# sakarias88/racer-tracer

Measured on AMD Instinct MI355X. Metric: Msamples/s (W*H*spp/s) at 1920x1080, higher is better.
Workload: dtype f64; 1 GPU; cornell_box.yml 1920x1080 1024spp max_depth 20; strip_rows=8, parallelism=image rows interleaved over 1 GPU(s)

## Files before the change

racer-tracer_amd/csrc/rt_pool_lds.h:

```cpp
#pragma once
#include "rt_trace_common.h"

namespace RT_KNS {

struct NoiseSlots {
    double p[8][3];
    int depth[8];
    int perlin[8];
    double term[8][8];
};
struct alignas(16) Req4 {
    uint32_t x, y, z, w;
};
struct alignas(8) SphereSlot {
    uint32_t b, y, x, w, z, base;
};
static_assert(sizeof(SphereSlot) == 3 * sizeof(double), "a slot holds the request or the sample");

template <bool TEXTURED> union SamplerScratch {
    Req4 req[32];
    SphereSlot sphere[32];
    NoiseSlots noise;
};
template <> union SamplerScratch<false> {
    Req4 req[32];
    SphereSlot sphere[32];
};

struct alignas(16) ItemInfo {
    int chunk, tx, ty, tile_py0, region, reg_tiles, rows_aligned, _pad;
};

template <bool TEXTURED, int NBUF, bool OVERLAP> struct WaveLds {
    double base[OVERLAP ? 1 : 64][3];
    double u[OVERLAP ? 64 : 1];
    double sum[OVERLAP ? 128 : 64][3];
    SamplerScratch<TEXTURED> scratch;
    uint8_t pix_of[64];
    double v[NBUF][64];
    ItemInfo info[2];
    double ulc[3];
};

enum : uint32_t { RING_SLOTS = 92u };
struct PretraceLds {
    double cam_origin[3], bg_top[3];
    double u[64];
    double sum[64][3];
    SamplerScratch<false> scratch;
    uint8_t pix_of[64];
    double ring_v[RING_SLOTS];
    double ring_t[RING_SLOTS];
    uint32_t ring_w[RING_SLOTS];
    uint16_t ring_best[RING_SLOTS];
    uint32_t n_started;
    uint32_t rect_mask;
    ItemInfo info[1];
    double ulc[3];
};

}
```

racer-tracer_amd/csrc/rt_trace_common.h:

```cpp
#pragma once
#include <hip/hip_runtime.h>
#include <stdint.h>
#include "rt_device_types.h"
#include "rt_bvh_slab.h"
#include "../../include/rt_abi.h"
#include "../../include/rt_rng.h"

#ifdef RT_EXACT_DIV
#define RT_KNS rtdev_exact
#define RT_LAUNCHER(name) name##_exact
#else
#define RT_KNS rtdev_fast
#define RT_LAUNCHER(name) name
#endif

namespace RT_KNS {
using namespace rtdev;

#define RT_CONSTANT __attribute__((address_space(4)))
__device__ __forceinline__ Prim load_prim_uniform(const Prim *table, int i) {
    Prim p;
    __builtin_memcpy(&p, (const RT_CONSTANT Prim *)(table + i), sizeof(Prim));
    return p;
}
// ... 340 lines not shown
#ifndef RT_EXACT_DIV
        return box_slab_t(P.p, o, d, inv_d, t_min, t_max, t_out, aux);
#endif
        bool any = false;
        double closest = t_max;
#pragma unroll
        for (int s = 0; s < 6; ++s) {
            int axis;
            double a0, a1, b0, b1, k, t;
            box_side(P.p, s, axis, a0, a1, b0, b1, k);
            if (rect_t<false>(axis, a0, a1, b0, b1, k, o, d, inv_d, t_min, closest, t)) {
                closest = t;
                aux = s;
                any = true;
            }
        }
        t_out = closest;
        return any;
    }
    }
}

__device__ __forceinline__ bool box_t(const Prim &P, d3 o, d3 d, d3 inv_d, double t_min, double t_max, double &t_out, int &side) {
#ifdef RT_EXACT_DIV
    return prim_t<PRIMS_ANY>(P, o, d, inv_d, 0.0, 0.0, t_min, t_max, t_out, side);
#else
#ifndef RT_BOX_LOADS_LAZY
    asm volatile("; box record requested" ::"s"(P.p[0]), "s"(P.p[1]), "s"(P.p[2]), "s"(P.p[3]), "s"(P.p[4]), "s"(P.p[5]), "s"(P.rot_sin),
                 "s"(P.rot_cos), "s"(P.tr[0]), "s"(P.tr[1]), "s"(P.tr[2]), "s"(P.flags));
#endif
    o = o - ld3(P.tr);
    if (P.flags & RT_PRIM_HAS_ROTATE_Y) {
        o = rot_fwd(o, P.rot_sin, P.rot_cos);
        d = rot_fwd(d, P.rot_sin, P.rot_cos);
        inv_d.x = rcp_f64(d.x);
        inv_d.z = rcp_f64(d.z);
    }
    return box_slab_t(P.p, o, d, inv_d, t_min, t_max, t_out, side);
#endif
}

__device__ __forceinline__ const BvhNode *bvh_nodes_for(const TraceArgs &A, d3 d) {
    if (A.bvh_nodes_ordered == nullptr) return A.bvh_nodes;
    const int oct = (d.x < 0.0 ? 1 : 0) | (d.y < 0.0 ? 2 : 0) | (d.z < 0.0 ? 4 : 0);
    return A.bvh_nodes_ordered + (size_t)oct * (size_t)(A.n_bvh_nodes + 1);
}

struct NoMark {
    __device__ __forceinline__ void operator()(int) const {}
};
template <int PRIMS, class Mark = NoMark>
__device__ __forceinline__ void closest_hit_bvh(const TraceArgs &A, const BvhNode *nodes, d3 o, d3 d, d3 inv_d,
                                                double inv_a, double time, double t_min, double &best_t, int &best,
                                                int &best_aux, unsigned *walk_stats = nullptr, Mark mark = Mark()) {
    const RT_CONSTANT TraceArgs *K = kernargs_here();
    double t0 = 0.0;
    {
        const double ax = (K->bvh_root_mn[0] - o.x) * inv_d.x, bx = (K->bvh_root_mx[0] - o.x) * inv_d.x;
        const double ay = (K->bvh_root_mn[1] - o.y) * inv_d.y, by = (K->bvh_root_mx[1] - o.y) * inv_d.y;
        const double az = (K->bvh_root_mn[2] - o.z) * inv_d.z, bz = (K->bvh_root_mx[2] - o.z) * inv_d.z;
        const double t_enter = fmax(fmax(fmin(ax, bx), fmin(ay, by)), fmin(az, bz));
        const double t_exit = fmin(fmin(fmax(ax, bx), fmax(ay, by)), fmin(fmax(az, bz), best_t));
        if (!(fmax(t_enter, t_min) <= t_exit)) return;
        if (t_enter > 0.0) t0 = t_enter;
    }
    const SlabRay sr = slab_ray((float)(fma(t0, d.x, o.x) - K->bvh_center[0]), (float)(fma(t0, d.y, o.y) - K->bvh_center[1]),
                                (float)(fma(t0, d.z, o.z) - K->bvh_center[2]), inv_d.x, inv_d.y, inv_d.z);
    const float slack = 0x1p-20f;
    const float tmin_f = (float)(t_min - t0) - fabsf((float)(t_min - t0)) * slack - 0x1p-126f;
    auto far_of = [&](double bt) {
        const float f = (float)(bt - t0);
        return fmaxf(f + fabsf(f) * slack, tmin_f);
    };
    float best_f = far_of(best_t);
    if (!(tmin_f <= best_f)) return;
    typedef float f2 __attribute__((ext_vector_type(2)));
    const f2 p01 = {sr.ivx, sr.ivy}, p23 = {sr.ivz, sr.nox}, p45 = {sr.noy, sr.noz};
    int i = 0;
    const int n = A.n_bvh_nodes;
    while (i < n) {
        int fc = 0;
        for (;;) {
            if (walk_stats) ++walk_stats[0];
            const uint4 *raw = reinterpret_cast<const uint4 *>(&nodes[i]);
            const uint4 q0 = raw[0], q1 = raw[1];
            const f2 qx = {__uint_as_float(q0.x), __uint_as_float(q0.y)}, qy = {__uint_as_float(q0.z), __uint_as_float(q0.w)},
                     qz = {__uint_as_float(q1.x), __uint_as_float(q1.y)};
            f2 tx, ty, tz;
            float nx, ny, nz, fx, fy, fz, t_near, t_far;
            asm("v_pk_fma_f32 %0, %1, %2, %3 op_sel:[0,0,1] op_sel_hi:[1,0,1]" : "=v"(tx) : "v"(qx), "v"(p01), "v"(p23));
            asm("v_pk_fma_f32 %0, %1, %2, %3 op_sel:[0,1,0] op_sel_hi:[1,1,0]" : "=v"(ty) : "v"(qy), "v"(p01), "v"(p45));
            asm("v_pk_fma_f32 %0, %1, %2, %3 op_sel:[0,0,1] op_sel_hi:[1,0,1]" : "=v"(tz) : "v"(qz), "v"(p23), "v"(p45));
            asm("v_min_f32 %0, %8, %9\n\tv_max_f32 %1, %8, %9\n\t"
                "v_min_f32 %2, %10, %11\n\tv_max_f32 %3, %10, %11\n\t"
                "v_min_f32 %4, %12, %13\n\tv_max_f32 %5, %12, %13\n\t"
                "v_max_f32 %4, %4, %14\n\tv_min_f32 %5, %5, %15\n\t"
                "v_max3_f32 %6, %0, %2, %4\n\tv_min3_f32 %7, %1, %3, %5"
                : "=&v"(nx), "=&v"(fx), "=&v"(ny), "=&v"(fy), "=&v"(nz), "=&v"(fz), "=&v"(t_near), "=&v"(t_far)
                : "v"(tx.x), "v"(tx.y), "v"(ty.x), "v"(ty.y), "v"(tz.x), "v"(tz.y), "v"(tmin_f), "v"(best_f));
            const bool hit = !(t_near > t_far);
            fc = (int)q1.w;
            i = hit ? i + 1 : (int)q1.z;
            if (hit && fc != 0) break;
        }
        const int count = fc & 7, first = fc >> 3;
        mark(11);
        bool improved = false;
        for (int k = 0; k < count; ++k) {
            if (walk_stats) ++walk_stats[1];
            const int pi = first + k;
            double t;
            int aux = 0;
            bool hit;
            const LeafGeo &G = A.leaf_geo[pi];
            const long long tag = G.tag;
            const d3 center = ld3(G.c0) + ((time - A.leaf_time_a) * A.leaf_inv_dt) * ld3(G.dc);
            hit = sphere_t(center, G.radius2, o, d, inv_a, t_min, best_t, t) && tag == 0;
            if (tag != 0) hit = prim_t<PRIMS>(A.prims[pi], o, d, inv_d, inv_a, time, t_min, best_t, t, aux);
            if (hit) {
                best_t = t;
                best = pi;
                best_aux = aux;
                improved = true;
            }
        }
        if (improved) best_f = far_of(best_t);
        mark(12);
    }
}

struct UV {
    double u, v;
};
__device__ __noinline__ UV sphere_uv(d3 outward) {
    const double PI = 3.14159265358979323846;
    double theta = acos(-outward.y);
    double phi = atan2(-outward.z, outward.x) + PI;
#ifdef RT_EXACT_DIV
    return UV{phi / (2.0 * PI), theta / PI};
#else
    return UV{phi * (1.0 / (2.0 * PI)), theta * (1.0 / PI)};
#endif
}

#define RT_UV_EPS_U 5e-7
#define RT_UV_EPS_V 2e-6
__device__ __forceinline__ UV sphere_uv_f32(d3 outward) {
    const float theta = acosf(-(float)outward.y);
    const float phi = atan2f(-(float)outward.z, (float)outward.x);
    return UV{((double)phi + 3.14159265358979323846) * (1.0 / (2.0 * 3.14159265358979323846)),
              (double)theta * (1.0 / 3.14159265358979323846)};
}

template <int PRIMS, bool TEXTURED, bool FAST_UV = false>
__device__ __forceinline__ Hit prim_hit_record(const Prim &P, d3 o, d3 d, double time, double t, int aux, bool want_uv) {
    d3 oo = o, dd = d;
    const int flags = PRIMS == PRIMS_ANY ? P.flags : 0;
    if (flags & RT_PRIM_HAS_TRANSLATE) oo = oo - ld3(P.tr);
    if (flags & RT_PRIM_HAS_ROTATE_Y) {
        oo = rot_fwd(oo, P.rot_sin, P.rot_cos);
        dd = rot_fwd(dd, P.rot_sin, P.rot_cos);
    }
    Hit h;
    h.point = oo + t * dd;
    h.u = 0.0;
    h.v = 0.0;
    h.uv_approx = false;
    const int kind = PRIMS == PRIMS_SPHERES ? (int)RT_PRIM_SPHERE : P.kind;
    if (PRIMS == PRIMS_ANY && kind == RT_PRIM_MOVING_SPHERE) {
        const d3 center = ld3(P.p) + ((time - P.rot_sin) * P.rot_cos) * ld3(P.tr);
        d3 outward = (h.point - center) * P.inv_radius;
        if (TEXTURED && want_uv) {
            const UV uv = sphere_uv(h.point);
            h.u = uv.u;
            h.v = uv.v;
        }
        set_face_normal(h, dd, outward);
    } else if (PRIMS != PRIMS_RECTS && kind == RT_PRIM_SPHERE) {
        d3 outward = (h.point - ld3(P.p)) * P.inv_radius;
        if (TEXTURED && want_uv) {
#ifndef RT_EXACT_DIV
            if (FAST_UV && flags == 0 && fma(-outward.y, outward.y, 1.0) >= 0x1p-10) {
                const UV uv = sphere_uv_f32(outward);
                h.u = uv.u;
                h.v = uv.v;
                h.uv_approx = true;
            } else
#endif
            {
                const UV uv = sphere_uv(outward);
                h.u = uv.u;
                h.v = uv.v;
            }
        }
        set_face_normal(h, dd, outward);
    } else {
        int axis;
        double a0, a1, b0, b1, k;
        if (PRIMS == PRIMS_ANY && kind == RT_PRIM_BOX) {
            box_side(P.p, aux, axis, a0, a1, b0, b1, k);
        } else {
            axis = kind == RT_PRIM_XY_RECT ? 2 : (kind == RT_PRIM_XZ_RECT ? 1 : 0);
            a0 = P.p[0]; a1 = P.p[1]; b0 = P.p[2]; b1 = P.p[3];
        }
        if (TEXTURED && want_uv) {
            int ia = axis == 0 ? 1 : 0;
            int ib = axis == 2 ? 1 : 2;
            h.u = (comp(h.point, ia) - a0) / (a1 - a0);
            h.v = (comp(h.point, ib) - b0) / (b1 - b0);
        }
        set_face_normal_axis(h, dd, axis);
    }
    if (flags & RT_PRIM_HAS_ROTATE_Y) {
        h.point = rot_back(h.point, P.rot_sin, P.rot_cos);
        set_face_normal(h, dd, rot_back(h.normal, P.rot_sin, P.rot_cos));
    }
    if (flags & RT_PRIM_HAS_TRANSLATE) {
        h.point = h.point + ld3(P.tr);
        set_face_normal(h, d, h.normal);
    }
    return h;
}

template <bool IDENTITY>
__device__ __forceinline__ double perlin_noise(const Perlin &pl, d3 p) {
    double fx = floor(p.x), fy = floor(p.y), fz = floor(p.z);
    double u = p.x - fx, v = p.y - fy, w = p.z - fz;
    int i = (int)fx, j = (int)fy, k = (int)fz;
    double uu = u * u * (3.0 - 2.0 * u);
    double vv = v * v * (3.0 - 2.0 * v);
    double ww = w * w * (3.0 - 2.0 * w);
    const double fu[2] = {1.0 - uu, uu}, fv[2] = {1.0 - vv, vv}, fw[2] = {1.0 - ww, ww};
    double accum = 0.0;
#pragma unroll
    for (int di = 0; di < 2; ++di)
#pragma unroll
        for (int dj = 0; dj < 2; ++dj) {
            const double fuv = fu[di] * fv[dj];
#pragma unroll
            for (int dk = 0; dk < 2; ++dk) {
                int index;
                if (IDENTITY)
                    index = (i + di) ^ (j + dj) ^ (k + dk);
                else
                    index = pl.perm_x[(uint32_t)(i + di) & 255u] ^ pl.perm_y[(uint32_t)(j + dj) & 255u] ^
                            pl.perm_z[(uint32_t)(k + dk) & 255u];
                const double *g = pl.ranvec[index & 255];
                d3 weight = mk(u - di, v - dj, w - dk);
                accum += fuv * fw[dk] * dot(ld3(g), weight);
            }
        }
    return accum;
}

template <bool IDENTITY>
__device__ __forceinline__ double perlin_turbulence(const Perlin &pl, d3 p, int depth) {
    double accum = 0.0, weight = 1.0;
    for (int o = 0; o < depth; ++o) {
        accum += weight * perlin_noise<IDENTITY>(pl, p);
        weight *= 0.5;
        p = p * 2.0;
    }
    return fabs(accum);
}

__device__ __forceinline__ double clamp01(double x) { return x < 0.0 ? 0.0 : (x > 1.0 ? 1.0 : x); }

__device__ __forceinline__ double sin_lean(double x) {
    const double kd = rint(x * 0.63661977236758134308);
    double r = fma(-kd, 1.57079632673412561417e+00, x);
    r = fma(-kd, 6.07710050630396597660e-11, r);
    r = fma(-kd, 2.02226624871116645580e-21, r);
    const int q = (int)kd;
    const double z = r * r;
    const double ps = fma(z, fma(z, fma(z, fma(z, 1.58969099521155010221e-10, -2.50507602534068634195e-08),
                                        2.75573137070700676789e-06), -1.98412698298579493134e-04),
                          8.33333333332248946124e-03);
    const double sn = fma(z * r, fma(z, ps, -1.66666666666666324348e-01), r);
    const double pc = fma(z, fma(z, fma(z, fma(z, fma(z, -1.13596475577881948265e-11, 2.08757232129817482790e-09),
                                               -2.75573143513906633035e-07), 2.48015872894767294178e-05),
                                 -1.38888888888741095749e-03), 4.16666666666666019037e-02);
    const double cs = 1.0 - fma(0.5, z, -(z * z) * pc);
    const double v = (q & 1) ? cs : sn;
    return (q & 2) ? -v : v;
}

__device__ __forceinline__ int sin_sign(double x) {
    const double kd = rint(x * 0.63661977236758134308);
    double r = fma(-kd, 1.57079632673412561417e+00, x);
    r = fma(-kd, 6.07710050630396597660e-11, r);
    r = fma(-kd, 2.02226624871116645580e-21, r);
    const int q = (int)kd;
    const int s = (q & 1) ? 1 : (r > 0.0 ? 1 : (r < 0.0 ? -1 : 0));
    return (q & 2) ? -s : s;
}

__device__ __forceinline__ bool sines_product_negative(double a, double b, double c) {
#ifndef RT_EXACT_DIV
    const double inv_pi = 0.31830988618379067154;
    const uint32_t odd = (uint32_t)(int)floor(a * inv_pi) ^ (uint32_t)(int)floor(b * inv_pi) ^ (uint32_t)(int)floor(c * inv_pi);
    const bool zero = a * b * c == 0.0;
    return !zero && (odd & 1u) != 0u;
#else
    uint32_t negative = 0;
    bool zero = false;
    const double xs[3] = {a, b, c};
#pragma unroll
    for (int k = 0; k < 3; ++k) {
        const double kd = rint(xs[k] * 0.63661977236758134308);
        double r = fma(-kd, 1.57079632673412561417e+00, xs[k]);
        r = fma(-kd, 6.07710050630396597660e-11, r);
        r = fma(-kd, 2.02226624871116645580e-21, r);
        const uint32_t q = (uint32_t)(int)kd;
        const uint32_t r_neg = (uint32_t)((unsigned long long)__double_as_longlong(r) >> 63);
        zero = zero || ((q & 1u) == 0u && r == 0.0);
        negative ^= (q >> 1) ^ (~q & r_neg);
    }
// ... 95 lines not shown
```

racer-tracer_amd/csrc/rt_trace_pool_kernel.hip:

```cpp
#include <cstddef>
#include <type_traits>
#include "rt_trace_common.h"
#include "rt_primary_bounds.h"
#include "rt_variant_dispatch.h"
#include "rt_pool_profile.h"
#include "rt_pool_lds.h"
#include "rt_pool_coop.h"
#include "rt_pool_deliver.h"

#ifndef RT_OCC_TEX
#define RT_OCC_TEX 4
#endif
#ifndef RT_OCC_TEX_BVH
#define RT_OCC_TEX_BVH 4
#endif
#ifndef RT_OCC_TEX_ANY
#define RT_OCC_TEX_ANY 4
#endif
#ifndef RT_OCC_SPEC
#define RT_OCC_SPEC 5
#endif
#ifndef RT_OCC_ANY
#define RT_OCC_ANY 5
#endif
// ... 171 lines not shown
        const uint64_t valid_mask = ballot(my_valid);
        n_valid = __popcll(valid_mask);
        bool culled = false;
        if constexpr (PRETRACE) {
            const RT_CONSTANT TraceArgs *K = kernargs_here();
            const int x0 = K->cull_px0, x1 = K->cull_px1, y0 = K->cull_py0, y1 = K->cull_py1;
            const uint64_t seen = valid_mask & ballot(my_px >= x0) & ballot(my_px <= x1) & ballot(my_py >= y0) & ballot(my_py <= y1);
            culled = seen == 0ull && K->bg.kind != RT_BG_SKY && K->max_depth >= 1;
            uint32_t rect_mask = ~0u;
            if (!culled) {
                const RT_CONSTANT rtdev::PrimaryRects *R = primary_rects_here();
                const int n_rects = R->n;
                for (int i = 0; i < n_rects; ++i) {
                    const int rx0 = R->r[i].px0, rx1 = R->r[i].px1, ry0 = R->r[i].py0, ry1 = R->r[i].py1;
                    const uint64_t sees = valid_mask & ballot(my_px >= rx0) & ballot(my_px <= rx1) & ballot(my_py >= ry0) & ballot(my_py <= ry1);
                    if (sees == 0ull) rect_mask &= ~(1u << i);
                }
            }
            if (lane == 0) L.rect_mask = rect_mask;
        }
        {
            if (!culled) {
                uint32_t pixel_stream = RT_RNG_SAMPLE_PIXEL;
                if constexpr (PRETRACE) asm volatile("" : "+s"(pixel_stream));
                PathRng prng{my_pixel, pixel_stream, A.seed_lo, A.seed_hi};
                u4 bj = prng.block(0, RT_RNG_PIXEL, 0);
                const RT_CONSTANT TraceArgs *K = kernargs_here();
                const double u = div_by((double)my_px + u53(bj.a, bj.b), (double)(A.width - 1), K->inv_width_m1);
                if constexpr (OVERLAP || PRETRACE) {
                    L.u[lane] = u;
                } else {
                    const d3 base = ld3(K->cam.ulc) + u * ld3(K->cam.horizontal);
                    L.base[lane][0] = base.x;
                    L.base[lane][1] = base.y;
                    L.base[lane][2] = base.z;
                }
            }
            unsigned long long zero = FIXED_SUMS ? 0ull - (unsigned long long)n_smp * 0x4330000000000000ull : 0ull;
            if constexpr (PRETRACE) asm volatile("" : "+v"(zero));
            unsigned long long *sum = reinterpret_cast<unsigned long long *>(L.sum[cur * 64 + lane]);
            sum[0] = zero;
            sum[1] = zero;
            sum[2] = zero;
            if (my_valid) L.pix_of[lane_rank(valid_mask)] = lane;
            if (lane == 0) L.info[cur] = ItemInfo{(int)chunk, tx, ty, tile_py0, region, (int)reg_tiles, rows_aligned ? 1 : 0, 0};
        }
        if constexpr (PRETRACE) {
            if (culled) {
                const d3 bg = ld3(L.bg_top);
                if (bg.x != 0.0 || bg.y != 0.0 || bg.z != 0.0)
                    for (int k = 0; k < n_smp; ++k) {
                        atomicAdd(&L.sum[lane_of_wave][0], bg.x);
                        atomicAdd(&L.sum[lane_of_wave][1], bg.y);
                        atomicAdd(&L.sum[lane_of_wave][2], bg.z);
                    }
                if (__builtin_amdgcn_inverse_ballot_w64(valid_mask)) n_segments += (unsigned int)n_smp;
                if (lane == 0) L.n_started += (uint32_t)n_valid * (uint32_t)n_smp;
            }
        }
        if (!rows_aligned) tile_py0 = -1;
        total = culled ? 0u : (uint32_t)n_valid * (uint32_t)n_smp;
        next = 0;
        n_batches = (total + 63u) >> 6;
        batches_done = 0;
        batch_due = n_batches > 0u ? 0u : ~0u;
        ring_head = 0;
        return true;
    };
    auto finish_item = [&](int s) {
        int lane = lane_of_wave;
        asm volatile("" : "+v"(lane));
        const ItemInfo I = L.info[s];
        const int chunk = __builtin_amdgcn_readfirstlane(I.chunk), f_tx = __builtin_amdgcn_readfirstlane(I.tx),
                  f_ty = __builtin_amdgcn_readfirstlane(I.ty), f_py0 = __builtin_amdgcn_readfirstlane(I.tile_py0);
        const bool f_aligned = __builtin_amdgcn_readfirstlane(I.rows_aligned) != 0;
        const int f_px = (f_tx * 8 + (lane & 7)) * A.step_x;
        const int f_vrow = f_ty * 8 + (lane >> 3);
        int f_py = f_py0 + (lane >> 3) * A.step_y;
        if (!f_aligned) f_py = ((f_vrow / A.strip_rows) * A.strip_count + A.strip_index) * A.strip_rows + f_vrow % A.strip_rows;
        const bool f_valid = f_px < A.cover_w && f_vrow < A.owned_rows && f_py < A.height;
        double s0 = L.sum[s * 64 + lane][0], s1 = L.sum[s * 64 + lane][1], s2 = L.sum[s * 64 + lane][2];
        if (FIXED_SUMS) {
            const double unscale = kernargs_here()->sum_unscale;
            s0 = (double)(unsigned long long)__double_as_longlong(s0) * unscale;
            s1 = (double)(unsigned long long)__double_as_longlong(s1) * unscale;
            s2 = (double)(unsigned long long)__double_as_longlong(s2) * unscale;
        }
        if (A.deliver_out == nullptr) {
            if (f_valid) {
                const size_t in_slice = (size_t)f_vrow * (size_t)A.width + (size_t)f_px;
                double *dst = A.partial + ((size_t)(A.chunk_base + chunk) * (size_t)A.slice_rows * (size_t)A.width + in_slice) * 3;
                dst[0] = s0;
                dst[1] = s1;
                dst[2] = s2;
            }
        } else {
            deliver_item(kernargs_here(), s0, s1, s2, f_valid, chunk, f_tx, f_ty, f_py0, f_aligned, __builtin_amdgcn_readfirstlane(I.region),
                         (uint32_t)__builtin_amdgcn_readfirstlane(I.reg_tiles));
        }
    };
    auto entry_of = [&](uint32_t w, int &py_out, uint32_t &pixel_out, uint32_t &sample_out, int &pix) {
        int s_off;
        if (n_valid == 64) {
            pix = (int)(w & 63u);
            s_off = (int)(w >> 6);
        } else {
            s_off = (int)(w / (uint32_t)n_valid);
            pix = L.pix_of[w - (uint32_t)s_off * (uint32_t)n_valid];
        }
        pixel_out = (uint32_t)shfl_i((int)my_pixel, pix);
        py_out = tile_py0 + (pix >> 3) * A.step_y;
        if (tile_py0 < 0) {
            const int vrow = __builtin_amdgcn_readfirstlane(L.info[(state >> 6) & 1u].ty) * 8 + (pix >> 3);
            py_out = ((vrow / A.strip_rows) * A.strip_count + A.strip_index) * A.strip_rows + vrow % A.strip_rows;
        }
        sample_out = (uint32_t)(smp0 + s_off);
    };
    auto prepare_batch = [&](uint32_t b) {
        if constexpr (!PRETRACE) {
        int lane = lane_of_wave;
        asm volatile("" : "+v"(lane));
        const RT_CONSTANT TraceArgs *K = kernargs_here();
        const uint32_t w = b * 64u + (uint32_t)lane;
        const bool in_pool = w < total;
        int py_b = 0;
        uint32_t pixel_b = 0, sample_b = 0;
        int pix_b = 0;
        entry_of(w, py_b, pixel_b, sample_b, pix_b);
        const u4 bc = philox4x32(pixel_b, sample_b, RT_RNG_CAMERA, 0u, A.seed_lo, A.seed_hi);
        const int buf = (int)(b & (uint32_t)(NBUF - 1));
        L.v[buf][lane] = div_by((double)py_b + u53(bc.a, bc.b), (double)(A.height - 1), K->inv_height_m1);
        if (PRIMS == PRIMS_ANY && ray_times != nullptr) ray_times[buf][lane] = K->cam.time_a + (K->cam.time_b - K->cam.time_a) * u53(bc.c, bc.d);
        if (K->cam.lens_radius != 0.0) {
            double lx = 0.0, ly = 0.0;
            coop_random_in_unit_disk(in_pool, pixel_b, sample_b, A.seed_lo, A.seed_hi, lane, L.scratch.req, lx, ly);
            lens[buf][lane][0] = lx * K->cam.lens_radius;
            lens[buf][lane][1] = ly * K->cam.lens_radius;
        }
        }
    };

    auto camera_ray = [&](int pix, double v, double lens_x, double lens_y, d3 &ro, d3 &rd) {
        if constexpr (PRETRACE) {
        const RT_CONSTANT TraceArgs *K = kernargs_here();
        ro = ld3(L.cam_origin);
        rd = (ld3(L.ulc) + L.u[pix] * ld3(K->cam.horizontal)) - v * ld3(K->cam.vertical) - ld3(K->cam.origin);
        if (kernargs_here()->lens_lds != 0) {
            const d3 offset = ld3(K->cam.right) * lens_x + ld3(K->cam.up) * lens_y;
            ro = ro + offset;
            rd = rd - offset;
        }
        }
    };
    double (*const lens_ring)[2] = reinterpret_cast<double (*)[2]>(lens);
    static_assert(RING_SLOTS <= 2 * 64, "the ring's lens samples take the LDS of two batches'");
    auto pretrace_batch = [&](uint32_t b) {
        if constexpr (PRETRACE) {
        int lane = lane_of_wave;
        asm volatile("" : "+v"(lane));
        const RT_CONSTANT TraceArgs *K = kernargs_here();
        const uint32_t w = b * 64u + (uint32_t)lane;
        const uint64_t in_pool = ballot(w < total);
        int py_b = 0, pix_b = 0;
        uint32_t pixel_b = 0, sample_b = 0;
        entry_of(w, py_b, pixel_b, sample_b, pix_b);
        const int max_depth = K->max_depth;
        if (max_depth <= 0) {
            double one = 1.0;
            asm volatile("" : "+v"(one));
            if (__builtin_amdgcn_inverse_ballot_w64(in_pool)) {
                atomicAdd(&L.sum[pix_b][0], one);
                atomicAdd(&L.sum[pix_b][1], one);
                atomicAdd(&L.sum[pix_b][2], one);
            }
            if (lane == 0) L.n_started += (uint32_t)__popcll(in_pool);
            next += (uint32_t)__popcll(in_pool);
            return;
        }
        const u4 bc = philox4x32(pixel_b, sample_b, RT_RNG_CAMERA, 0u, A.seed_lo, A.seed_hi);
        const uint32_t in_ring = min(b << 6, total) - next;
        uint32_t park = ring_head + in_ring + (uint32_t)lane;
        if (park >= RING_SLOTS) park -= RING_SLOTS;
        d3 bo, bd;
        {
            const double v = div_by((double)py_b + u53(bc.a, bc.b), (double)(A.height - 1), K->inv_height_m1);
            double lx, ly;
            asm volatile("" : "=v"(lx), "=v"(ly));
            if (kernargs_here()->lens_lds != 0) {
                lx = ly = 0.0;
                uint32_t w_here = w;
                asm volatile("" : "+v"(w_here));
                coop_random_in_unit_disk(w_here < total, pixel_b, sample_b, A.seed_lo, A.seed_hi, lane, L.scratch.req, lx, ly);
                lx = lx * K->cam.lens_radius;
                ly = ly * K->cam.lens_radius;
                lens_ring[park][0] = lx;
                lens_ring[park][1] = ly;
            }
            L.ring_v[park] = v;
            camera_ray(pix_b, v, lx, ly, bo, bd);
        }
        double best_t = __builtin_inf();
        int best = -1;
        increment_masked(n_segments, in_pool);
        const uint32_t rect_mask = (uint32_t)__builtin_amdgcn_readfirstlane((int)L.rect_mask);
        closest_hit_rects<false>(A.prims, bo, bd, rcp3(bd), best_t, best, rect_mask);
        d3 C = ld3(L.bg_top);
        if (kernargs_here()->bg.kind == RT_BG_SKY) {
            const double t = 0.5 * (unit_fast(bd).y + 1.0);
            C = (1.0 - t) * C + t * ld3(kernargs_here()->bg.bottom);
        }
        const uint64_t hit = in_pool & ballot(best >= 0);
        int kind;
        asm volatile("" : "=v"(kind));
        if (__builtin_amdgcn_inverse_ballot_w64(hit)) {
            const Material &M = lds_prims[best].mat;
            kind = M.kind;
            C = ld3(M.color);
        }
        asm volatile("" : "+v"(kind));
        const uint64_t light = hit & ballot(kind == RT_MAT_DIFFUSE_LIGHT);
        const uint64_t ends = kernargs_here()->max_depth <= 1 ? in_pool : (in_pool & ~hit) | light;
        const uint64_t lives = in_pool & ~ends;
        if (__builtin_amdgcn_inverse_ballot_w64(ends)) {
            double *const sum = reinterpret_cast<double *>(reinterpret_cast<unsigned char *>(&L.sum[0][0]) + (uint32_t)pix_b * (uint32_t)sizeof(L.sum[0]));
            atomicAdd(sum + 0, C.x);
            atomicAdd(sum + 1, C.y);
            atomicAdd(sum + 2, C.z);
        }
        if (lane == 0) L.n_started += (uint32_t)__popcll(in_pool);
        uint32_t slot = ring_head + in_ring + (uint32_t)lane_rank(lives);
        if (slot >= RING_SLOTS) slot -= RING_SLOTS;
        if (__builtin_amdgcn_inverse_ballot_w64(lives)) {
            const double v = L.ring_v[park];
            double lx, ly;
            asm volatile("" : "=v"(lx), "=v"(ly));
            if (kernargs_here()->lens_lds != 0) {
                lx = lens_ring[park][0];
                ly = lens_ring[park][1];
            }
            asm volatile("" ::: "memory");
            L.ring_v[slot] = v;
            L.ring_t[slot] = best_t;
            L.ring_w[slot] = w;
            L.ring_best[slot] = (uint16_t)best;
            if (kernargs_here()->lens_lds != 0) {
                lens_ring[slot][0] = lx;
                lens_ring[slot][1] = ly;
            }
        }
        next += (uint32_t)__popcll(ends);
        }
    };

    uint64_t alive_m = 0;
    int spix = 0;
    PathRng rng{0, 0, A.seed_lo, A.seed_hi};
    d3 o = mk(0, 0, 0), d = o, T = o;
    uint32_t seg = 0;
    double ray_time = 0.0;
    uint64_t waiting_m = 0;
    uint32_t cand_base = 0;
    uint64_t lambert_m = 0;
    d3 hit_normal = o;
    double fuzz = 0.0;

    for (;;) {
        if ((state & (HAVE | DRAINING)) == HAVE && next >= total) {
            state ^= HAVE | DRAINING | (OVERLAP ? CUR : 0u);
            state &= ~POOL_DRY;
            total = next = n_batches = batches_done = 0;
            batch_due = ~0u;
        }
        if ((state & DRAINING) != 0u && (OVERLAP ? alive_m & ballot((((uint32_t)spix ^ state) & CUR) != 0u) : alive_m) == 0) {
            finish_item(OVERLAP ? (int)((state ^ CUR) >> 6) & 1 : 0);
            state &= ~DRAINING;
        }
        if ((state & (HAVE | QUEUE_DRY)) == 0u && (FIXED_SUMS || (state & DRAINING) == 0u)) {
            state |= start_item() ? HAVE : QUEUE_DRY;
            if (OVERLAP && (state & HAVE) != 0u && total == 0u) state |= POOL_DRY;
        }
        if ((state & (HAVE | DRAINING)) == 0u) break;
        RT_REGION(0);
        if (!OVERLAP) {
            alive_m = waiting_m = lambert_m = 0;
            spix = 0;
            rng.pixel = rng.sample = 0;
            o = d = T = hit_normal = mk(0, 0, 0);
            seg = cand_base = 0;
            ray_time = fuzz = 0.0;
        }
        if constexpr (PRETRACE) {
            double best_t = __builtin_inf();
            int best = -1;
            for (;;) {
                while (batches_done < n_batches && min(batches_done << 6, total) - next <= RING_SLOTS - 64u) pretrace_batch(batches_done++);
                RT_REGION(1);
                const uint32_t in_ring = min(batches_done << 6, total) - next;
                if (in_ring != 0u) {
                    const uint64_t idle = ~alive_m;
                    const uint32_t r = (uint32_t)lane_rank(idle);
                    uint32_t slot = ring_head + r;
                    if (slot >= RING_SLOTS) slot -= RING_SLOTS;
                    const uint32_t w = L.ring_w[slot];
                    int s_off, pix_new;
                    if (n_valid == 64) {
                        pix_new = (int)(w & 63u);
                        s_off = (int)(w >> 6);
                    } else {
                        s_off = (int)(w / (uint32_t)n_valid);
                        pix_new = L.pix_of[(w - (uint32_t)s_off * (uint32_t)n_valid) & 63u];
                    }
                    const uint32_t pixel_new = (uint32_t)shfl_i((int)my_pixel, pix_new);
                    const uint64_t taking = idle & ballot(r < in_ring);
                    const uint32_t n_take = min((uint32_t)__popcll(idle), in_ring);
                    next += n_take;
                    ring_head += n_take;
                    if (ring_head >= RING_SLOTS) ring_head -= RING_SLOTS;
                    if (__builtin_amdgcn_inverse_ballot_w64(taking)) {
                        spix = pix_new;
                        rng.pixel = pixel_new;
                        rng.sample = (uint32_t)(smp0 + s_off);
                        double lens_x, lens_y;
                        asm volatile("" : "=v"(lens_x), "=v"(lens_y));
                        if (kernargs_here()->lens_lds != 0) {
                            lens_x = lens_ring[slot][0];
                            lens_y = lens_ring[slot][1];
                        }
                        camera_ray(pix_new, L.ring_v[slot], lens_x, lens_y, o, d);
                        best_t = L.ring_t[slot];
                        best = (int)L.ring_best[slot];
                        T = mk(1.0, 1.0, 1.0);
                        seg = 0;
                    }
                    alive_m |= taking;
                }
                RT_REGION(2);
                if (alive_m == 0) break;
                uint64_t ended_m = 0;
                const uint64_t hit_m = alive_m & ~waiting_m;
                int kind;
                asm volatile("" : "=v"(kind));
                if (__builtin_amdgcn_inverse_ballot_w64(hit_m)) {
                    const Prim &P = lds_prims[best];
                    const Material &M = P.mat;
                    const Hit h = prim_hit_record<PRIMS, TEXTURED, true>(P, o, d, ray_time, best_t, 0, false);
                    kind = M.kind;
                    RT_REGION(8);
                    T = T * ld3(M.color);
                    RT_REGION(9);
                    o = h.point;
                    cand_base = 0;
#ifndef RT_EXACT_DIV
                    {
                        const int axis = P.kind == RT_PRIM_XY_RECT ? 2 : (P.kind == RT_PRIM_XZ_RECT ? 1 : 0);
                        auto against = [](double dk, bool on_axis) {
                            uint32_t lo = 0u;
                            asm volatile("" : "+v"(lo));
                            const uint32_t hi = on_axis ? 0xBFF00000u ^ ((uint32_t)((unsigned long long)__double_as_longlong(dk) >> 32) & 0x80000000u) : 0u;
                            return __longlong_as_double((long long)((unsigned long long)hi << 32 | lo));
                        };
                        const uint64_t xy_m = ballot(axis == 2), xz_m = ballot(axis == 1);
                        d = mk(against(d.x, __builtin_amdgcn_inverse_ballot_w64(~(xy_m | xz_m))), against(d.y, __builtin_amdgcn_inverse_ballot_w64(xz_m)),
                               against(d.z, __builtin_amdgcn_inverse_ballot_w64(xy_m)));
                    }
#else
                    d = h.normal;
#endif
                }
                asm volatile("" : "+v"(kind));
                const uint64_t light_m = hit_m & ballot(kind == RT_MAT_DIFFUSE_LIGHT);
                ended_m |= light_m;
                waiting_m |= hit_m & ~light_m;
                RT_REGION(4);
                d3 sph = mk(0.0, 0.0, 0.0);
                const uint64_t finish_m = coop_random_in_unit_sphere<2>(waiting_m, rng.pixel, rng.sample, seg, cand_base, A.seed_lo, A.seed_hi, lane,
                                                                        L.scratch.sphere, sph);
                waiting_m &= ~finish_m;
                RT_REGION(5);
                if (__builtin_amdgcn_inverse_ballot_w64(finish_m)) {
                    const d3 dir = d + unit_fast(sph);
                    const uint64_t near_zero = ballot(fabs(dir.x) < 1e-8) & ballot(fabs(dir.y) < 1e-8) & ballot(fabs(dir.z) < 1e-8);
#ifndef RT_EXACT_DIV
                    d = dir;
                    if (near_zero != 0) {
                        asm volatile("; near_zero (keeps the compiler from turning the branch back into selects)");
                        if ((near_zero >> lane) & 1ull) {
                            const d3 u = unit_fast(sph);
                            d = mk(rint(-u.x) + 0.0, rint(-u.y) + 0.0, rint(-u.z) + 0.0);
                        }
                    }
#else
                    const d3 normal = d;
                    d = dir;
                    if (near_zero != 0) {
                        asm volatile("; near_zero (keeps the compiler from turning the branch back into selects)");
                        if ((near_zero >> lane) & 1ull) d = normal;
                    }
#endif
                }
                increment_masked(seg, finish_m);
                const uint64_t deep_m = finish_m & ballot((int)seg >= A.max_depth);
                ended_m |= deep_m;
                const uint64_t shooting = finish_m & ~deep_m;
                RT_LANES(__popcll(shooting), next >= total);
                asm volatile("" : "=v"(best_t), "=v"(best));
                if (__builtin_amdgcn_inverse_ballot_w64(shooting)) {
                    best_t = __builtin_inf();
                    best = -1;
                    ++n_segments;
                    closest_hit_rects<true>(A.prims, o, d, rcp3(d), best_t, best);
                    RT_REGION(3);
                }
                const uint64_t miss_m = shooting & ballot(best < 0);
                uint64_t adding_m = ended_m;
                ended_m |= miss_m;
                if (kernargs_here()->bg_black == 0) {
                    adding_m = ended_m;
                    const RT_CONSTANT TraceArgs *K = kernargs_here();
                    const uint64_t sky_m = K->bg.kind == RT_BG_SKY ? miss_m : 0ull;
                    if (__builtin_amdgcn_inverse_ballot_w64(miss_m & ~sky_m)) {
                        T.x = T.x * K->bg.top[0];
                        T.y = T.y * K->bg.top[1];
                        T.z = T.z * K->bg.top[2];
                    }
                    if (__builtin_amdgcn_inverse_ballot_w64(sky_m)) {
                        const double t = 0.5 * (unit_fast(d).y + 1.0);
                        T = T * ((1.0 - t) * ld3(K->bg.top) + t * ld3(K->bg.bottom));
                    }
                }
                if (__builtin_amdgcn_inverse_ballot_w64(adding_m)) {
                    atomicAdd(&L.sum[spix][0], T.x);
                    atomicAdd(&L.sum[spix][1], T.y);
                    atomicAdd(&L.sum[spix][2], T.z);
                }
                alive_m &= ~ended_m;
                RT_REGION(6);
            }
        } else
        for (;;) {
        while (next >= batch_due) {
            prepare_batch(batches_done++);
            batch_due = batches_done >= n_batches ? ~0u : (batches_done < (uint32_t)NBUF ? 0u : (batches_done - (uint32_t)(NBUF - 1)) << 6);
        }
        RT_REGION(1);
        if (next < total) {
            const uint64_t idle = ~alive_m;
            const uint32_t w = next + (uint32_t)lane_rank(idle);
            const uint32_t ready = NBUF == 2 ? total : min(total, batches_done << 6);
            next = min(next + (uint32_t)__popcll(idle), ready);
            if (OVERLAP && next >= total) state |= POOL_DRY;
            int s_off, pix_new;
            if (n_valid == 64) {
                pix_new = (int)(w & 63u);
                s_off = (int)(w >> 6);
            } else {
                s_off = (int)(w / (uint32_t)n_valid);
                pix_new = L.pix_of[w - (uint32_t)s_off * (uint32_t)n_valid];
            }
            const uint32_t pixel_new = (uint32_t)shfl_i((int)my_pixel, pix_new);
            const uint64_t taking = idle & ballot(w < ready);
            if (__builtin_amdgcn_inverse_ballot_w64(taking)) {
                spix = (int)(state & CUR) | pix_new;
                rng.pixel = pixel_new;
                rng.sample = (uint32_t)(smp0 + s_off);
                const RT_CONSTANT TraceArgs *K = kernargs_here();
                const int buf = (int)((w >> 6) & (uint32_t)(NBUF - 1)), slot = (int)(w & 63u);
                const double v = L.v[buf][slot];
                const d3 co = ld3(K->cam.origin);
                o = co;
                if (OVERLAP) d = (ld3(L.ulc) + L.u[pix_new] * ld3(K->cam.horizontal)) - v * ld3(K->cam.vertical) - co;
                else d = ld3(L.base[pix_new]) - v * ld3(K->cam.vertical) - co;
                const double lr = K->cam.lens_radius;
                if (lr != 0.0) {
                    const d3 offset = ld3(K->cam.right) * lens[buf][slot][0] + ld3(K->cam.up) * lens[buf][slot][1];
                    o = co + offset;
                    d = d - offset;
                }
                if (PRIMS == PRIMS_ANY && ray_times != nullptr) ray_time = ray_times[buf][slot];
                T = mk(1.0, 1.0, 1.0);
                seg = 0;
                ++n_started;
            }
            alive_m |= taking;
        }
        RT_REGION(2);
        if (!OVERLAP && alive_m == 0) break;
        uint64_t ended_m = 0;
        uint64_t scattered_m = 0;
        uint64_t finish_m = 0;
        const uint64_t tracing = alive_m & ~waiting_m;
        int noise_tex = -1;
        RT_LANES(__popcll(tracing), next >= total);
        int max_depth = A.max_depth;
        asm volatile("" : "+s"(max_depth));
        const uint64_t shooting = max_depth <= 0 ? 0ull : tracing;
        ended_m = tracing & ~shooting;
        double best_t = __builtin_inf();
        int best = -1, best_aux = 0;
        int kind;
        asm volatile("" : "=v"(kind));
        {
            if (__builtin_amdgcn_inverse_ballot_w64(shooting)) {
                ++n_segments;
                const d3 inv_d = rcp3(d);
                const double inv_a = PRIMS == PRIMS_RECTS ? 0.0 : rcp_f64(len2(d));
                if (BVH) {
#ifdef RT_PROFILE_REGIONS
                    unsigned walk[2] = {0, 0};
                    unsigned *walk_stats = walk;
#else
                    unsigned *walk_stats = nullptr;
#endif
#ifdef RT_PROFILE_REGIONS
                    auto walk_mark = [&](int k) { RT_REGION(k); };
#else
                    const NoMark walk_mark;
#endif
                    if (lds_nodes != nullptr)
                        closest_hit_bvh<PRIMS>(A, lds_nodes, o, d, inv_d, inv_a, ray_time, 0.001, best_t, best, best_aux, walk_stats, walk_mark);
                    else
                        closest_hit_bvh<PRIMS>(A, bvh_nodes_for(A, d), o, d, inv_d, inv_a, ray_time, 0.001, best_t, best, best_aux, walk_stats, walk_mark);
#ifdef RT_PROFILE_REGIONS
                    atomicAdd(&rt_t_[37], (unsigned long long)walk[0]);
                    atomicAdd(&rt_t_[38], (unsigned long long)walk[1]);
#endif
                } else {
                    auto test = [&](const Prim &P, int i) {
                        double t;
                        int aux;
                        if (prim_t<PRIMS>(P, o, d, inv_d, inv_a, ray_time, 0.001, best_t, t, aux)) {
                            best_t = t;
                            best = i;
                            best_aux = aux;
                        }
                    };
                    if (PRIMS != PRIMS_SPHERES) {
                        auto test_plane = [&](auto axis, const Prim &P, int i) {
#ifndef RT_EXACT_DIV
                            rect_closest_update<decltype(axis)::value>(P.p[0], P.p[1], P.p[2], P.p[3], P.p[4], o, d, inv_d, 0.001, best_t, best, i);
                            return;
#endif
                            double t;
                            if (rect_t<true>(decltype(axis)::value, P.p[0], P.p[1], P.p[2], P.p[3], P.p[4], o, d, inv_d, 0.001, best_t, t)) {
                                best_t = t;
                                best = i;
                            }
                        };
                        const Prim *rec = A.prims;
                        int i = 0;
                        auto group = [&](auto axis, int end) {
                            for (; i + 1 < end; i += 2, rec += 2) {
                                const Prim pa = load_prim_uniform(rec, 0), pb = load_prim_uniform(rec, 1);
                                test_plane(axis, pa, i);
                                test_plane(axis, pb, i + 1);
                            }
                            if (i < end) {
                                test_plane(axis, load_prim_uniform(rec, 0), i);
                                ++i;
                                ++rec;
                            }
                        };
                        const RT_CONSTANT TraceArgs *KB = kernargs_here();
                        const int end_xy = KB->rect_end[0], end_xz = KB->rect_end[1], end_yz = KB->rect_end[2];
// ... 299 lines not shown
```

Baseline: 42750 Msamples/s.

## Store hit points and direction signs in pretrace ring instead of camera params

```diff
diff --git a/racer-tracer_amd/csrc/rt_pool_lds.h b/racer-tracer_amd/csrc/rt_pool_lds.h
--- a/racer-tracer_amd/csrc/rt_pool_lds.h
+++ b/racer-tracer_amd/csrc/rt_pool_lds.h
@@ -42,15 +42,15 @@
     double ulc[3];
 };
 
-enum : uint32_t { RING_SLOTS = 92u };
+enum : uint32_t { RING_SLOTS = 67u };
+enum : uint32_t { RING_BEST_BITS = 13u, RING_BEST_MASK = (1u << RING_BEST_BITS) - 1u };
 struct PretraceLds {
     double cam_origin[3], bg_top[3];
     double u[64];
     double sum[64][3];
     SamplerScratch<false> scratch;
     uint8_t pix_of[64];
-    double ring_v[RING_SLOTS];
-    double ring_t[RING_SLOTS];
+    double ring_p[3][RING_SLOTS];
     uint32_t ring_w[RING_SLOTS];
     uint16_t ring_best[RING_SLOTS];
     uint32_t n_started;
diff --git a/racer-tracer_amd/csrc/rt_trace_common.h b/racer-tracer_amd/csrc/rt_trace_common.h
--- a/racer-tracer_amd/csrc/rt_trace_common.h
+++ b/racer-tracer_amd/csrc/rt_trace_common.h
@@ -516,6 +516,8 @@
               (double)theta * (1.0 / 3.14159265358979323846)};
 }
 
+__device__ __forceinline__ d3 ray_at(d3 o, double t, d3 d) { return o + t * d; }
+
 template <int PRIMS, bool TEXTURED, bool FAST_UV = false>
 __device__ __forceinline__ Hit prim_hit_record(const Prim &P, d3 o, d3 d, double time, double t, int aux, bool want_uv) {
     d3 oo = o, dd = d;
@@ -526,7 +528,7 @@
         dd = rot_fwd(dd, P.rot_sin, P.rot_cos);
     }
     Hit h;
-    h.point = oo + t * dd;
+    h.point = ray_at(oo, t, dd);
     h.u = 0.0;
     h.v = 0.0;
     h.uv_approx = false;
diff --git a/racer-tracer_amd/csrc/rt_trace_pool_kernel.hip b/racer-tracer_amd/csrc/rt_trace_pool_kernel.hip
--- a/racer-tracer_amd/csrc/rt_trace_pool_kernel.hip
+++ b/racer-tracer_amd/csrc/rt_trace_pool_kernel.hip
@@ -347,8 +347,6 @@
         }
         }
     };
-    double (*const lens_ring)[2] = reinterpret_cast<double (*)[2]>(lens);
-    static_assert(RING_SLOTS <= 2 * 64, "the ring's lens samples take the LDS of two batches'");
     auto pretrace_batch = [&](uint32_t b) {
         if constexpr (PRETRACE) {
         int lane = lane_of_wave;
@@ -374,8 +372,6 @@
         }
         const u4 bc = philox4x32(pixel_b, sample_b, RT_RNG_CAMERA, 0u, A.seed_lo, A.seed_hi);
         const uint32_t in_ring = min(b << 6, total) - next;
-        uint32_t park = ring_head + in_ring + (uint32_t)lane;
-        if (park >= RING_SLOTS) park -= RING_SLOTS;
         d3 bo, bd;
         {
             const double v = div_by((double)py_b + u53(bc.a, bc.b), (double)(A.height - 1), K->inv_height_m1);
@@ -388,10 +384,7 @@
                 coop_random_in_unit_disk(w_here < total, pixel_b, sample_b, A.seed_lo, A.seed_hi, lane, L.scratch.req, lx, ly);
                 lx = lx * K->cam.lens_radius;
                 ly = ly * K->cam.lens_radius;
-                lens_ring[park][0] = lx;
-                lens_ring[park][1] = ly;
-            }
-            L.ring_v[park] = v;
+            }
             camera_ray(pix_b, v, lx, ly, bo, bd);
         }
         double best_t = __builtin_inf();
@@ -426,22 +419,16 @@
         uint32_t slot = ring_head + in_ring + (uint32_t)lane_rank(lives);
         if (slot >= RING_SLOTS) slot -= RING_SLOTS;
         if (__builtin_amdgcn_inverse_ballot_w64(lives)) {
-            const double v = L.ring_v[park];
-            double lx, ly;
-            asm volatile("" : "=v"(lx), "=v"(ly));
-            if (kernargs_here()->lens_lds != 0) {
-                lx = lens_ring[park][0];
-                ly = lens_ring[park][1];
-            }
-            asm volatile("" ::: "memory");
-            L.ring_v[slot] = v;
-            L.ring_t[slot] = best_t;
+            asm volatile("; hit_point_begin" : "+v"(best_t));
+            d3 p = ray_at(bo, best_t, bd);
+            asm volatile("; hit_point_end" : "+v"(p.x), "+v"(p.y), "+v"(p.z));
+            auto sign_of = [](double dk) { return (uint32_t)((unsigned long long)__double_as_longlong(dk) >> 63); };
+            L.ring_p[0][slot] = p.x;
+            L.ring_p[1][slot] = p.y;
+            L.ring_p[2][slot] = p.z;
             L.ring_w[slot] = w;
-            L.ring_best[slot] = (uint16_t)best;
-            if (kernargs_here()->lens_lds != 0) {
-                lens_ring[slot][0] = lx;
-                lens_ring[slot][1] = ly;
-            }
+            L.ring_best[slot] = (uint16_t)((uint32_t)best | sign_of(bd.x) << RING_BEST_BITS | sign_of(bd.y) << (RING_BEST_BITS + 1u) |
+                                           sign_of(bd.z) << (RING_BEST_BITS + 2u));
         }
         next += (uint32_t)__popcll(ends);
         }
@@ -485,7 +472,6 @@
             ray_time = fuzz = 0.0;
         }
         if constexpr (PRETRACE) {
-            double best_t = __builtin_inf();
             int best = -1;
             for (;;) {
                 while (batches_done < n_batches && min(batches_done << 6, total) - next <= RING_SLOTS - 64u) pretrace_batch(batches_done++);
@@ -512,20 +498,27 @@
                     ring_head += n_take;
                     if (ring_head >= RING_SLOTS) ring_head -= RING_SLOTS;
                     if (__builtin_amdgcn_inverse_ballot_w64(taking)) {
+                        asm volatile("; hand_out_begin");
                         spix = pix_new;
                         rng.pixel = pixel_new;
                         rng.sample = (uint32_t)(smp0 + s_off);
-                        double lens_x, lens_y;
-                        asm volatile("" : "=v"(lens_x), "=v"(lens_y));
-                        if (kernargs_here()->lens_lds != 0) {
-                            lens_x = lens_ring[slot][0];
-                            lens_y = lens_ring[slot][1];
-                        }
-                        camera_ray(pix_new, L.ring_v[slot], lens_x, lens_y, o, d);
-                        best_t = L.ring_t[slot];
-                        best = (int)L.ring_best[slot];
+                        o = mk(L.ring_p[0][slot], L.ring_p[1][slot], L.ring_p[2][slot]);
+                        uint32_t word = L.ring_best[slot];
+                        asm volatile("" : "+v"(word));
+                        best = (int)(word & RING_BEST_MASK);
+                        auto signed_like = [word](uint32_t k) {
+                            uint32_t lo;
+                            asm volatile("" : "=v"(lo));
+                            uint32_t hi = word << (31u - RING_BEST_BITS - k);
+#ifdef RT_EXACT_DIV
+                            hi = 0x3FF00000u | (hi & 0x80000000u);
+#endif
+                            return __longlong_as_double((long long)((unsigned long long)hi << 32 | lo));
+                        };
+                        d = mk(signed_like(0u), signed_like(1u), signed_like(2u));
                         T = mk(1.0, 1.0, 1.0);
                         seg = 0;
+                        asm volatile("; hand_out_end");
                     }
                     alive_m |= taking;
                 }
@@ -538,12 +531,10 @@
                 if (__builtin_amdgcn_inverse_ballot_w64(hit_m)) {
                     const Prim &P = lds_prims[best];
                     const Material &M = P.mat;
-                    const Hit h = prim_hit_record<PRIMS, TEXTURED, true>(P, o, d, ray_time, best_t, 0, false);
                     kind = M.kind;
                     RT_REGION(8);
                     T = T * ld3(M.color);
                     RT_REGION(9);
-                    o = h.point;
                     cand_base = 0;
 #ifndef RT_EXACT_DIV
                     {
@@ -559,7 +550,11 @@
                                against(d.z, __builtin_amdgcn_inverse_ballot_w64(xy_m)));
                     }
 #else
-                    d = h.normal;
+                    {
+                        Hit h;
+                        set_face_normal_axis(h, d, P.kind == RT_PRIM_XY_RECT ? 2 : (P.kind == RT_PRIM_XZ_RECT ? 1 : 0));
+                        d = h.normal;
+                    }
 #endif
                 }
                 asm volatile("" : "+v"(kind));
@@ -598,12 +593,15 @@
                 ended_m |= deep_m;
                 const uint64_t shooting = finish_m & ~deep_m;
                 RT_LANES(__popcll(shooting), next >= total);
-                asm volatile("" : "=v"(best_t), "=v"(best));
+                asm volatile("" : "=v"(best));
                 if (__builtin_amdgcn_inverse_ballot_w64(shooting)) {
-                    best_t = __builtin_inf();
+                    double best_t = __builtin_inf();
                     best = -1;
                     ++n_segments;
                     closest_hit_rects<true>(A.prims, o, d, rcp3(d), best_t, best);
+                    asm volatile("; hit_point_begin" : "+v"(best_t));
+                    o = ray_at(o, best_t, d);
+                    asm volatile("; hit_point_end" : "+v"(o.x), "+v"(o.y), "+v"(o.z));
                     RT_REGION(3);
                 }
                 const uint64_t miss_m = shooting & ballot(best < 0);
```

After: 43610 Msamples/s (median of 6 runs). 2.0% higher.
